# Vicky-Lamperouge/dlsa

Measured on AMD Instinct MI355X. Metric: DLSA logistic fit rows/sec (node), n=1e8 p=100, 1/2/4/8 GPUs; HBM GB/s, higher is better.
Workload: dtype f64

## Files before the change

### dlsa_amd/csrc/irls_oz_impl.hpp

```cpp
#pragma once

#include <stdint.h>
#include <stdlib.h>

#include <array>
#include <utility>

#include "dlsa_internal.hpp"
#include "wave_math.hpp"

namespace dlsa {

typedef int oz_i4 __attribute__((ext_vector_type(4)));

namespace ozk {

constexpr int NPW = 4;
constexpr int NCW = 4;
constexpr int RB = 32;
constexpr int RPW = RB / NPW;
constexpr int NSLOT = 6;
static_assert(NSLOT >= 6, "2 blocks in flight + 2 producing + 2 consuming");
#ifndef DLSA_OZ_CHECK
#define DLSA_OZ_CHECK 0
#endif
constexpr int ND = 5;
constexpr int GBITS = 38;
constexpr int NL = 5;
constexpr int EMIN = -985;
constexpr int EMAX = 1009;
constexpr double MAGIC = 6755399441055744.0 + 551911719040.0;

__host__ __device__ constexpr int xspan(int p) { return (RB * p * 8 + 16 + 15) & ~15; }
__host__ __device__ constexpr int npieces(int p) { return (xspan(p) + 1023) / 1024; }
__host__ __device__ constexpr int slot_bytes(int p) { return 16 + xspan(p) + 256; }
constexpr int kFeatBytes = 48;
constexpr int kMaxPiecesPerWave = 7;
__host__ __device__ constexpr int plane_off(int d) { return 8 * d; }
#ifndef DLSA_OZ_ABLATE
#define DLSA_OZ_ABLATE 0
#endif
__host__ __device__ constexpr int img_bytes(int NT) { return 16 * NT * kFeatBytes; }
__host__ __device__ constexpr int extra_bytes(int NT) { return 3 * 16 * NT * 8 + 16 * NT * 4; }
__host__ __device__ constexpr int lds_bytes(int NT, int p) {
  return NSLOT * slot_bytes(p) + extra_bytes(NT);
}
__host__ __device__ constexpr bool fits(int NT, int p) {
  return img_bytes(NT) <= RPW * p * 8 && lds_bytes(NT, p) <= 160 * 1024 &&
         npieces(p) <= NCW * kMaxPiecesPerWave;
}

constexpr unsigned strip_mask(int NT, int cw) {
  int load[NCW] = {0, 0, 0, 0};
  unsigned m[NCW] = {0, 0, 0, 0};
  for (int J = 0; J < NT; ++J) {
    int best = 0;
    for (int w = 1; w < NCW; ++w)
      if (load[w] < load[best]) best = w;
    load[best] += NT - J;
    m[best] |= 1u << J;
  }
  return m[cw];
}

template <int NT, int CW>
struct Tiles {
  static constexpr unsigned SM = strip_mask(NT, CW);
  static constexpr int count() {
    int c = 0;
    for (int J = 0; J < NT; ++J)
      if ((SM >> J) & 1u) c += NT - J;
    return c;
  }
  static constexpr int TW = count();
  static constexpr int index(int I, int J) {
    int c = 0;
    for (int j = 0; j < NT; ++j)
      if ((SM >> j) & 1u) {
        if (j == J) return c + (I - J);
        c += NT - j;
      }
    return -1;
  }
  static constexpr int I_of(int i) {
    for (int j = 0; j < NT; ++j)
      if ((SM >> j) & 1u) {
        if (i < NT - j) return j + i;
        i -= NT - j;
      }
    return -1;
  }
  static constexpr int J_of(int i) {
    for (int j = 0; j < NT; ++j)
      if ((SM >> j) & 1u) {
        if (i < NT - j) return j;
        i -= NT - j;
      }
    return -1;
  }
  static constexpr int strip_ordinal(int J) {
    int c = 0;
    for (int j = 0; j < J; ++j) c += (SM >> j) & 1u;
    return c;
  }
};

__device__ __forceinline__ uint32_t perm(uint32_t a, uint32_t b, uint32_t sel) {
  return __builtin_amdgcn_perm(a, b, sel);
}

__device__ __forceinline__ double level_value(const oz_i4 (&L)[NL], int r) {
  double v = (double)L[NL - 1][r];
#pragma unroll
  for (int k = NL - 2; k >= 0; --k) v = fma(v, 0x1p-8, (double)L[k][r]);
  return v;
}

__device__ __forceinline__ double xbound(uint32_t hi) {
  return __hiloint2double((int)(hi & 0x7FFFFFFFu), (int)0xFFFFFFFFu);
}
__device__ __forceinline__ int digit_exponent(uint32_t xhi, uint32_t zbits, double growth) {
  const double xb = xbound(xhi);
  const double zb = (double)__uint_as_float(zbits & 0x7FFFFFFFu) * (1.0 + 0x1p-16);
  double bound = fmax(fmax(zb, 0x1p-120), xb * 0x1p-60) * growth;
  bound = fmin(bound, 0.5 * xb);
  const int e = __builtin_amdgcn_frexp_exp(bound);
  return max(e, EMIN);
}
__device__ __forceinline__ bool digit_overflow(int e) { return e > EMAX; }

}

#ifdef DLSA_OZ_PROF
static __device__ unsigned long long g_oz_prof[32];
static inline int oz_prof_read_impl(unsigned long long* out) {
  if (hipDeviceSynchronize() != hipSuccess) return -1;
  if (hipMemcpyFromSymbol(out, HIP_SYMBOL(g_oz_prof), 32 * 8) != hipSuccess) return -1;
  unsigned long long z[32] = {0};
  return hipMemcpyToSymbol(HIP_SYMBOL(g_oz_prof), z, 32 * 8) == hipSuccess ? 0 : -1;
}
#define OZ_STAMP(v) const uint64_t v = __builtin_readcyclecounter()
#define OZ_STAMP_VAR(v) uint64_t v = 0
#define OZ_STAMP_SET(v) v = __builtin_readcyclecounter()
#define OZ_ADD(i, d) prof[i] += (d)
#define OZ_DECL uint64_t prof[4] = {0, 0, 0, 0}
#define OZ_FLUSH(base)                                                        \
  if (lane == 0)                                                              \
    for (int i_ = 0; i_ < 4; ++i_) atomicAdd(&g_oz_prof[(base) + i_], prof[i_])
#else
#define OZ_STAMP(v)
#define OZ_STAMP_VAR(v)
#define OZ_STAMP_SET(v)
#define OZ_ADD(i, d)
#define OZ_DECL
#define OZ_FLUSH(base)
#endif

template <int NT, int CW>
struct OzConsumer {
  using TL = ozk::Tiles<NT, CW>;
  static constexpr int TW = TL::TW;
  static constexpr int PMAX = 16 * NT;
  oz_i4 acc[TW > 0 ? TW : 1][ozk::NL];

  __device__ __forceinline__ void init() {
    static_for<(TW > 0 ? TW : 1)>([&](auto iI) {
      constexpr int i = decltype(iI)::value;
#pragma unroll
      for (int k = 0; k < ozk::NL; ++k) acc[i][k] = oz_i4{0, 0, 0, 0};
    });
  }

  template <typename Tick>
  __device__ __forceinline__ void consume(const char* xs, int p, int lane, Tick&& tick) {
    if constexpr (TW > 0) {
      const int i = lane & 15, g = lane >> 4;
      const char* im = xs + g * ozk::RPW * p * 8 + i * ozk::kFeatBytes;
      using u2 = unsigned __attribute__((ext_vector_type(2)));
      oz_i4 A0[2], A2[2];
      u2 A4[2];
      u2 Bd[2][ozk::ND];
      auto loadB = [&](auto jJ, int u) {
        constexpr int fo = 16 * decltype(jJ)::value * ozk::kFeatBytes;
#pragma unroll
        for (int b = 0; b < ozk::ND; ++b) Bd[u][b] = *(const u2*)(im + fo + 8 * b);
      };
      auto loadA = [&](auto tI, int u) {
        constexpr int fa = 16 * TL::I_of(decltype(tI)::value) * ozk::kFeatBytes;
        A0[u] = *(const oz_i4*)(im + fa);
        A2[u] = *(const oz_i4*)(im + fa + 16);
        A4[u] = *(const u2*)(im + fa + 32);
      };
      loadB(std::integral_constant<int, TL::J_of(0)>{}, 0);
      loadA(std::integral_constant<int, 0>{}, 0);
      static_for<TW>([&](auto tI) {
        constexpr int t = decltype(tI)::value;
        constexpr int J = TL::J_of(t);
        constexpr int ua = t & 1;
        constexpr int ub = TL::strip_ordinal(J) & 1;
        if constexpr (t + 1 < TW) {
          constexpr int Jn = TL::J_of(t + 1);
          if constexpr (Jn != J) loadB(std::integral_constant<int, Jn>{}, ub ^ 1);
          loadA(std::integral_constant<int, t + 1>{}, ua ^ 1);
        }
        __builtin_amdgcn_sched_barrier(0);
        const u2* d = Bd[ub];
        oz_i4 Bq[ozk::ND];
        Bq[0] = oz_i4{(int)d[0].x, (int)d[0].y, 0, 0};
#pragma unroll
        for (int b = 1; b < ozk::ND; ++b)
          Bq[b] = oz_i4{(int)d[b].x, (int)d[b].y, (int)d[b - 1].x, (int)d[b - 1].y};
        const oz_i4 a0 = A0[ua], a2 = A2[ua];
        const oz_i4 a4 = oz_i4{(int)A4[ua].x, (int)A4[ua].y, 0, 0};
        acc[t][0] = __builtin_amdgcn_mfma_i32_16x16x64_i8(a0, Bq[0], acc[t][0], 0, 0, 0);
        acc[t][1] = __builtin_amdgcn_mfma_i32_16x16x64_i8(a0, Bq[1], acc[t][1], 0, 0, 0);
        acc[t][2] = __builtin_amdgcn_mfma_i32_16x16x64_i8(a0, Bq[2], acc[t][2], 0, 0, 0);
        acc[t][3] = __builtin_amdgcn_mfma_i32_16x16x64_i8(a0, Bq[3], acc[t][3], 0, 0, 0);
        acc[t][4] = __builtin_amdgcn_mfma_i32_16x16x64_i8(a0, Bq[4], acc[t][4], 0, 0, 0);
        acc[t][2] = __builtin_amdgcn_mfma_i32_16x16x64_i8(a2, Bq[0], acc[t][2], 0, 0, 0);
        acc[t][3] = __builtin_amdgcn_mfma_i32_16x16x64_i8(a2, Bq[1], acc[t][3], 0, 0, 0);
        acc[t][4] = __builtin_amdgcn_mfma_i32_16x16x64_i8(a2, Bq[2], acc[t][4], 0, 0, 0);
        acc[t][4] = __builtin_amdgcn_mfma_i32_16x16x64_i8(a4, Bq[0], acc[t][4], 0, 0, 0);
        __builtin_amdgcn_sched_barrier(0);
        tick(std::integral_constant<int, t>{});
      });
      static_for<TW>([this](auto iI) {
        constexpr int t = decltype(iI)::value;
#pragma unroll
        for (int k = 0; k < ozk::NL; ++k) asm volatile("" : "+v"(acc[t][k]));
      });
    }
  }

  __device__ __forceinline__ void store(double* sH, const int* ex, int lane) {
    if constexpr (TW > 0) {
      const int fl = lane & 15, q = lane >> 4;
      static_for<TW>([&](auto iI) {
        constexpr int t = decltype(iI)::value;
        constexpr int I = TL::I_of(t), J = TL::J_of(t);
        constexpr int ts = I * (I + 1) / 2 + J;
        const int ej = ex[16 * J + fl];
#pragma unroll
        for (int r = 0; r < 4; ++r) {
          const int row = 4 * q + r;
          const double v = ozk::level_value(acc[t], r);
          sH[ts * 256 + row * 16 + fl] = __builtin_amdgcn_ldexp(v, ej + ex[16 * I + row] - 12);
        }
      });
    }
  }
};

template <int NT, bool STD, typename SlotX, typename Dma>
__device__ __forceinline__ void oz_producer(const PassArgs& a, char* smem, int wid, int lane,
                                            int tid, int nb, int nit, int sbytes, int xs_bytes,
                                            SlotX&& slot_x, const double* bet,
                                            const double* stdv, const int* ex, int chunk,
                                            bool chunk_ovf, Dma&& issue_pair) {
  using namespace ozk;
  constexpr int PMAX = 16 * NT;
  const int p = a.p, P = a.P, ic = a.intercept;
  const int nrows = __builtin_amdgcn_readfirstlane(a.chunk_rows[blockIdx.x]);
  const int pw = wid;
  const int q = lane >> 4, s = lane & 15;
  const int Xq = q >> 1, hq = q & 1;
  const int rbase = pw * RPW + 4 * hq;
  const bool up8 = s >= 8, up4 = ((s >> 2) & 1) != 0;
  const int myrow = s >> 2;
  double beta[NT], gacc[NT], mg[NT];
#pragma unroll
  for (int k = 0; k < NT; ++k) {
    const int f = 16 * k + s;
    beta[k] = bet[f];
    mg[k] = __builtin_amdgcn_ldexp(MAGIC, ex[f] - GBITS);
    gacc[k] = 0.0;
  }
  const bool fin_last = 16 * (NT - 1) + s < P;
  double llacc = 0.0, lprod = 1.0;

  issue_pair(-1);
  wait_vmcnt<0>();
  OZ_DECL;
  for (int m = 0; m < nit; ++m) {
    OZ_STAMP(t0);
    wait_vmcnt<0>();
    lds_barrier();
    OZ_STAMP(t1);
    OZ_ADD(0, t1 - t0);
    issue_pair(m);
    if (2 * m >= nb || (DLSA_OZ_ABLATE & 1)) continue;
    const int b = 2 * m + Xq;
    char* xq = slot_x(b);
    const double* yq = (const double*)(smem + (b % NSLOT) * sbytes + 16 + xs_bytes);
    const int leftq = nrows - b * RB;
    const bool full = nrows - 2 * m * RB >= 2 * RB;
    double v[4][NT], e[4];
    auto row_phase = [&](auto maskI) {
      constexpr bool MASK = decltype(maskI)::value;
#pragma unroll
      for (int r = 0; r < 4; ++r) {
        const int rowB = rbase + r;
        const bool valid = rowB < leftq;
        const double* xr = (const double*)xq + rowB * p + (s - ic);
        double er = 0.0;
#pragma unroll
        for (int k = 0; k < NT; ++k) {
          const int f = 16 * k + s;
          double x = xr[16 * k];
          if constexpr (DLSA_OZ_CHECK) {
            const int el = rowB * p + f - ic;
            if (f >= ic && f < P && (el < pw * RPW * p || el >= (pw + 1) * RPW * p))
              x = __builtin_nan("");
          }
          if constexpr (STD) x = (x - stdv[f]) * stdv[PMAX + f];
          if (k == 0 && ic && s == 0) x = 1.0;
          const bool fin = k < NT - 1 || fin_last;
          if constexpr (MASK)
            x = (valid && fin) ? x : 0.0;
          else
            x = fin ? x : 0.0;
          v[r][k] = x;
          er = fma(x, beta[k], er);
        }
        e[r] = er;
      }
    };
    if (full)
      row_phase(std::false_type{});
    else
      row_phase(std::true_type{});
    double e01, e23;
    {
      const double s0 = up8 ? e[0] : e[2], s1 = up8 ? e[1] : e[3];
      const double k0 = up8 ? e[2] : e[0], k1 = up8 ? e[3] : e[1];
      e01 = k0 + dpp_f64<0x128>(s0);
      e23 = k1 + dpp_f64<0x128>(s1);
    }
    double eh;
    {
      const double sn = up4 ? e01 : e23, kp = up4 ? e23 : e01;
      eh = kp + dpp_f64<0x141>(sn);
    }
    eh += dpp_f64<0xB1>(eh);
    eh += dpp_f64<0x4E>(eh);
    double swh, rh;
    {
      const bool valid = rbase + myrow < leftq;
      const double yv = valid ? yq[rbase + myrow] : 0.0;
      const double eqv = exp(-0.5 * fabs(eh));
      const double ea = eqv * eqv;
      const double inv = wv_rcp(1.0 + ea);
      const double mu = eh >= 0.0 ? inv : ea * inv;
      swh = eqv * inv;
      rh = yv - mu;
      if (valid && (s & 3) == 0) {
        llacc += yv * eh - fmax(eh, 0.0);
        lprod *= 1.0 + ea;
      }
      if (!valid) {
        swh = 0.0;
        rh = 0.0;
      }
    }
    double sw[4], res[4];
    sw[0] = dpp_f64<0x150>(swh);
    sw[1] = dpp_f64<0x154>(swh);
    sw[2] = dpp_f64<0x158>(swh);
    sw[3] = dpp_f64<0x15C>(swh);
    res[0] = dpp_f64<0x150>(rh);
    res[1] = dpp_f64<0x154>(rh);
    res[2] = dpp_f64<0x158>(rh);
    res[3] = dpp_f64<0x15C>(rh);
    OZ_STAMP(t2);
    OZ_ADD(1, t2 - t1);
    char* img = xq + pw * RPW * p * 8 + 4 * hq;
#pragma unroll
    for (int k = 0; k < NT; ++k) {
      gacc[k] = fma(v[0][k], res[0], gacc[k]);
      gacc[k] = fma(v[1][k], res[1], gacc[k]);
      gacc[k] = fma(v[2][k], res[2], gacc[k]);
      gacc[k] = fma(v[3][k], res[3], gacc[k]);
      uint32_t lo[4], hi[4];
#pragma unroll
      for (int r = 0; r < 4; ++r) {
        const double t = fma(v[r][k], sw[r], mg[k]);
        lo[r] = __double2loint(t);
        hi[r] = __double2hiint(t);
      }
      const uint32_t u01 = perm(lo[1], lo[0], 0x05010400u), w01 = perm(lo[1], lo[0], 0x07030602u);
      const uint32_t u23 = perm(lo[3], lo[2], 0x05010400u), w23 = perm(lo[3], lo[2], 0x07030602u);
      const uint32_t d4 = perm(u23, u01, 0x05040100u) ^ 0x80808080u;
      const uint32_t d3 = perm(u23, u01, 0x07060302u) ^ 0x80808080u;
      const uint32_t d2 = perm(w23, w01, 0x05040100u) ^ 0x80808080u;
      const uint32_t d1 = perm(w23, w01, 0x07060302u) ^ 0x80808080u;
      const uint32_t d0 = perm(perm(hi[3], hi[2], 0x05010400u), perm(hi[1], hi[0], 0x05010400u),
                               0x05040100u) ^ 0x80808080u;
      char* fe = img + (16 * k + s) * kFeatBytes;
      *(uint32_t*)(fe + plane_off(0)) = d0;
      *(uint32_t*)(fe + plane_off(1)) = d1;
      *(uint32_t*)(fe + plane_off(2)) = d2;
      *(uint32_t*)(fe + plane_off(3)) = d3;
      *(uint32_t*)(fe + plane_off(4)) = d4;
    }
#ifdef DLSA_OZ_PROF
    asm volatile("s_waitcnt lgkmcnt(0)" ::: "memory");
#endif
    OZ_STAMP(t3);
    OZ_ADD(2, t3 - t2);
  }
  OZ_FLUSH(4 * pw);
  __syncthreads();

  double* red = (double*)smem;
#pragma unroll
  for (int k = 0; k < NT; ++k) {
    double g = gacc[k];
    g += __shfl_xor(g, 16);
    g += __shfl_xor(g, 32);
    if (q == 0) red[pw * (PMAX + 1) + 16 * k + s] = g;
  }
  llacc -= log(lprod);
#pragma unroll
  for (int o = 1; o < 64; o <<= 1) llacc += __shfl_xor(llacc, o);
  if (lane == 0) red[pw * (PMAX + 1) + PMAX] = llacc;
  __syncthreads();
  for (int f = tid; f < PMAX; f += 64 * NPW) {
    double sg = 0.0;
#pragma unroll
    for (int w = 0; w < NPW; ++w) sg += red[w * (PMAX + 1) + f];
    a.slab_g[(int64_t)chunk * PMAX + f] = sg;
  }
  if (tid == 0) {
    double sg = 0.0;
#pragma unroll
    for (int w = 0; w < NPW; ++w) sg += red[w * (PMAX + 1) + PMAX];
    a.slab_ll[chunk] = chunk_ovf ? __builtin_nan("") : sg;
  }
}

template <int NT, bool STD>
__global__ __launch_bounds__(64 * (ozk::NPW + ozk::NCW), 1) void irls_oz_kernel(const PassArgs a) {
  using namespace ozk;
  constexpr int PMAX = 16 * NT;
  extern __shared__ __attribute__((aligned(16))) char smem[];

  const int chunk = blockIdx.x;
  const int part = __builtin_amdgcn_readfirstlane(a.chunk_part[chunk]);
  if (a.phase[part] != a.want_phase) return;

  const int tid = threadIdx.x;
  const int lane = tid & 63;
  const int wid = __builtin_amdgcn_readfirstlane(tid >> 6);
  const int p = a.p, P = a.P, ic = a.intercept;
  const int64_t row0 = uniform_row0(a.chunk_row0, chunk);
  const int nrows = __builtin_amdgcn_readfirstlane(a.chunk_rows[chunk]);
  const int nb = (nrows + RB - 1) / RB;
  const int nit = (nb + 1) / 2 + 1;
  const int sbytes = slot_bytes(p);
  const int np = npieces(p);
  const int xs_bytes = xspan(p);
  double* bet = (double*)(smem + NSLOT * sbytes);
  double* stdv = bet + PMAX;
  int* ex = (int*)(stdv + 2 * PMAX);

  double dth = 0.0;
  uint32_t xh = 0;
  bool e_ovf = false;
  if (tid < PMAX) {
    const double th = (tid < P) ? a.theta[(int64_t)part * P + tid] : 0.0;
    bet[tid] = th;
    if (tid < P) dth = fabs(th - a.theta_rec[(int64_t)part * P + tid]);
    xh = a.colmax[(int64_t)chunk * PMAX + tid] & 0x7FFFFFFFu;
    if constexpr (STD) {
      const int j = tid - ic;
      const bool in = j >= 0 && j < p;
      stdv[tid] = in ? a.center[j] : 0.0;
      stdv[PMAX + tid] = in ? 1.0 / a.scale[j] : 1.0;
    }
  }
#pragma unroll
  for (int o = 1; o < 64; o <<= 1) {
    dth += __shfl_xor(dth, o);
    xh = max(xh, (uint32_t)__shfl_xor((int)xh, o));
  }
  double* dred = (double*)smem;
  uint32_t* xred = (uint32_t*)(dred + (NPW + NCW));
  if (lane == 0) {
    dred[wid] = dth;
    xred[wid] = xh;
  }
  __syncthreads();
  if (tid < PMAX) {
    double sd = 0.0;
    uint32_t xm = 0;
#pragma unroll
    for (int w = 0; w < NPW + NCW; ++w) {
      sd += dred[w];
      xm = max(xm, xred[w]);
    }
    const double growth = exp(0.5 * sd * ozk::xbound(xm)) * (1.0 + 0x1p-40);
    const int e = digit_exponent(a.colmax[(int64_t)chunk * PMAX + tid],
                                 a.zcolmax[(int64_t)chunk * PMAX + tid], growth);
    ex[tid] = min(e, ozk::EMAX);
    if (wid == 0) {
      e_ovf = ozk::digit_overflow(e);
      if (tid + 64 < PMAX)
        e_ovf = e_ovf || ozk::digit_overflow(digit_exponent(
                             a.colmax[(int64_t)chunk * PMAX + tid + 64],
                             a.zcolmax[(int64_t)chunk * PMAX + tid + 64], growth));
    }
  }
  const bool chunk_ovf = wid == 0 && __ballot(e_ovf) != 0;
  __syncthreads();

  auto slot_x = [&](int blk) -> char* {
    const uintptr_t start = (uintptr_t)(a.X + (row0 + (int64_t)blk * RB) * p);
    return smem + (blk % NSLOT) * sbytes + 16 + (start & 15);
  };

  constexpr int KP = 1;
  const int dw = wid >= NPW ? wid - NPW : wid;
  const uintptr_t xcb = (uintptr_t)(a.X + row0 * p) & ~(uintptr_t)15;
  const __amdgpu_buffer_rsrc_t xr = uniform_rsrc(xcb, a.x_last16 + 16 - xcb);
  const uintptr_t ycb = (uintptr_t)(a.y + row0);
  const __amdgpu_buffer_rsrc_t yr = uniform_rsrc(ycb, a.y_last4 + 4 - ycb);
  const int npw = (np - dw + NCW - 1) / NCW;
  auto blk_lds = [&](int blk) { return __builtin_amdgcn_readfirstlane((blk % NSLOT) * sbytes); };
  auto blk_soff = [&](int blk) {
    const uintptr_t start = (uintptr_t)(a.X + (row0 + (int64_t)blk * RB) * p);
    return __builtin_amdgcn_readfirstlane((int)((start & ~(uintptr_t)15) - xcb));
  };
  auto issue_x = [&](auto iI, int lds, int soff) {
    constexpr int i = decltype(iI)::value;
    if (i < npw) {
      const int j = dw + NCW * i;
      const int off = j == np - 1 ? xs_bytes - 1024 : j * 1024;
      __builtin_amdgcn_raw_ptr_buffer_load_lds(xr, (lds_void_t*)(smem + lds + 16 + off), 16,
                                               lane * 16, soff + off, 0, DLSA_OZ_DMA_AUX);
    }
  };
  auto issue_y = [&](int blk, int lds) {
    if (dw == NCW - 1)
      __builtin_amdgcn_raw_ptr_buffer_load_lds(yr, (lds_void_t*)(smem + lds + 16 + xs_bytes), 4,
                                               lane * 4, blk * RB * 8, 0, 0);
  };
  auto issue_rest = [&](auto I0, int blk, int lds, int soff) {
    static_for<kMaxPiecesPerWave>([&](auto iI) {
      if constexpr (decltype(iI)::value >= decltype(I0)::value) issue_x(iI, lds, soff);
    });
    issue_y(blk, lds);
  };
  static_assert(KP == 1, "issue_pair issues piece 0 only");
  auto issue_pair = [&](int m) {
#pragma unroll
    for (int X = 2; X < 4; ++X) {
      const int blk = 2 * m + X;
      if (blk < nb) issue_x(std::integral_constant<int, 0>{}, blk_lds(blk), blk_soff(blk));
    }
  };

  if (wid >= NPW) {
    const int cw = wid - NPW;
    auto run = [&](auto cwI) {
      constexpr int CW = decltype(cwI)::value;
      constexpr int TW = OzConsumer<NT, CW>::TW;
      __builtin_amdgcn_s_setprio(1);
      OzConsumer<NT, CW> C;
      C.init();
      for (int b = 0; b < 2 && b < nb; ++b)
        issue_rest(std::integral_constant<int, KP>{}, b, blk_lds(b), blk_soff(b));
      wait_vmcnt<0>();
      OZ_DECL;
      for (int m = 0; m < nit; ++m) {
        OZ_STAMP(t0);
        lds_barrier();
        OZ_STAMP(t1);
        const bool d0 = 2 * m + 2 < nb, d1 = 2 * m + 3 < nb;
        const int l0 = blk_lds(2 * m + 2), s0 = blk_soff(2 * m + 2);
        const int l1 = blk_lds(2 * m + 3), s1 = blk_soff(2 * m + 3);
        const bool c0 = m >= 1 && !(DLSA_OZ_ABLATE & 2);
        const bool c1 = c0 && 2 * m - 1 < nb;
        OZ_STAMP_VAR(t2);
        auto tickA = [&](auto tI) {
          constexpr int i = KP + decltype(tI)::value;
          if (d0) issue_x(std::integral_constant<int, i>{}, l0, s0);
          if (d1) issue_x(std::integral_constant<int, i>{}, l1, s1);
        };
        auto tickN = [&](auto) {};
        if (c0) C.consume(slot_x(2 * m - 2), p, lane, tickA);
        if (c0) {
          if (d0) issue_rest(std::integral_constant<int, KP + TW>{}, 2 * m + 2, l0, s0);
          if (d1) issue_rest(std::integral_constant<int, KP + TW>{}, 2 * m + 3, l1, s1);
        } else {
          if (d0) issue_rest(std::integral_constant<int, KP>{}, 2 * m + 2, l0, s0);
          if (d1) issue_rest(std::integral_constant<int, KP>{}, 2 * m + 3, l1, s1);
        }
        if (c1) C.consume(slot_x(2 * m - 1), p, lane, tickN);
        OZ_STAMP_SET(t2);
        OZ_STAMP(t3);
        wait_vmcnt<0>();
        OZ_STAMP(t4);
        OZ_ADD(0, t1 - t0);
        OZ_ADD(1, t3 - t2);
        OZ_ADD(2, t2 - t1);
        OZ_ADD(3, t4 - t3);
      }
      OZ_FLUSH(4 * (NPW + CW));
      __syncthreads();
      C.store(a.slab_H + (int64_t)chunk * (NT * (NT + 1) / 2) * 256, ex, lane);
      __syncthreads();
    };
    switch (cw) {
      case 0: run(std::integral_constant<int, 0>{}); break;
      case 1: run(std::integral_constant<int, 1>{}); break;
      case 2: run(std::integral_constant<int, 2>{}); break;
      default: run(std::integral_constant<int, 3>{}); break;
    }
    return;
  }

  oz_producer<NT, STD>(a, smem, wid, lane, tid, nb, nit, sbytes, xs_bytes, slot_x, bet, stdv,
                       ex, chunk, chunk_ovf, issue_pair);
}

template <int NT, bool STD>
static hipError_t launch_oz_t(const PassArgs& a, int n_chunks, hipStream_t s) {
  auto kern = irls_oz_kernel<NT, STD>;
  hipError_t e = ensure_max_lds((const void*)kern, 160 * 1024);
  if (e != hipSuccess) return e;
  hipLaunchKernelGGL(kern, dim3(n_chunks), dim3(64 * (ozk::NPW + ozk::NCW)),
                     ozk::lds_bytes(NT, a.p), s, a);
  return hipGetLastError();
}

template <int NT>
static hipError_t launch_oz_nt(const PassArgs& a, bool std_, int n_chunks, hipStream_t s) {
  return std_ ? launch_oz_t<NT, true>(a, n_chunks, s) : launch_oz_t<NT, false>(a, n_chunks, s);
}

typedef hipError_t OzUnitFn(const PassArgs& a, int NT, bool std_, int family, int n_chunks,
                            hipStream_t s);
#define DLSA_OZ_UNIT(name, ...)                                                                  \
  hipError_t name(const PassArgs& a, int NT, bool std_, int family, int n_chunks, hipStream_t s) { \
    return unit_dispatch(FamLogistic{}, IntList<__VA_ARGS__>{}, family, NT, [&](auto, auto nt) { \
      return launch_oz_nt<decltype(nt)::value>(a, std_, n_chunks, s);                            \
    });                                                                                          \
  }

}
```

Before: 1.328 billion.

## Consume two row blocks per MFMA pass by pairing slots into 128-bit operands

The consumer now reads each digit plane from two adjacent LDS slots with explicit ds_read_b64 pairs and packs them into one 128-bit MFMA operand, so a single consume call covers both blocks of the pair instead of two separate consume calls. The MFMA product list is rewritten for full 5x5 digit pairs up to total order 4, and lgkmcnt waits are made explicit. The prefetch schedule issues four pieces up front (KP=4) instead of one. This aims to halve consume overhead and improve MFMA K utilisation, at the cost of more registers and hand-written asm waits that bypass compiler scheduling.

```diff
diff --git a/dlsa_amd/csrc/irls_oz_impl.hpp b/dlsa_amd/csrc/irls_oz_impl.hpp
--- a/dlsa_amd/csrc/irls_oz_impl.hpp
+++ b/dlsa_amd/csrc/irls_oz_impl.hpp
@@ -172,24 +172,41 @@
   }
 
   template <typename Tick>
-  __device__ __forceinline__ void consume(const char* xs, int p, int lane, Tick&& tick) {
+  __device__ __forceinline__ void consume(const char* xs, int sb, int p, int lane, Tick&& tick) {
     if constexpr (TW > 0) {
       const int i = lane & 15, g = lane >> 4;
       const char* im = xs + g * ozk::RPW * p * 8 + i * ozk::kFeatBytes;
+      const char* im1 = im + sb;
       using u2 = unsigned __attribute__((ext_vector_type(2)));
-      oz_i4 A0[2], A2[2];
-      u2 A4[2];
-      u2 Bd[2][ozk::ND];
+      const uint32_t a0 = (uint32_t)(uintptr_t)(const lds_void_t*)im, a1 = a0 + sb;
+      oz_i4 Ad[2][ozk::ND], Bd[2][ozk::ND];
+      auto plane = [&](auto offI) {
+        constexpr int off = decltype(offI)::value;
+        static_assert(off >= 0 && off < 65536, "ds_read_b64 takes a 16-bit byte offset");
+        u2 e, o;
+        asm volatile("ds_read_b64 %0, %1 offset:%2" : "=v"(e) : "v"(a0), "n"(off) : "memory");
+        asm volatile("ds_read_b64 %0, %1 offset:%2" : "=v"(o) : "v"(a1), "n"(off) : "memory");
+        return oz_i4{(int)e.x, (int)e.y, (int)o.x, (int)o.y};
+      };
+      auto load_planes = [&](oz_i4* q, auto foI) {
+        static_for<ozk::ND>([&](auto dI) {
+          constexpr int d = decltype(dI)::value;
+          q[d] = plane(std::integral_constant<int, decltype(foI)::value + ozk::plane_off(d)>{});
+        });
+      };
+      auto wait_planes = [&](oz_i4* a, oz_i4* b) {
+        static_assert(ozk::ND == 5, "the operand list below");
+        asm volatile("s_waitcnt lgkmcnt(0)"
+                     : "+v"(a[0]), "+v"(a[1]), "+v"(a[2]), "+v"(a[3]), "+v"(a[4]), "+v"(b[0]),
+                       "+v"(b[1]), "+v"(b[2]), "+v"(b[3]), "+v"(b[4]));
+      };
       auto loadB = [&](auto jJ, int u) {
-        constexpr int fo = 16 * decltype(jJ)::value * ozk::kFeatBytes;
-#pragma unroll
-        for (int b = 0; b < ozk::ND; ++b) Bd[u][b] = *(const u2*)(im + fo + 8 * b);
+        load_planes(Bd[u],
+                    std::integral_constant<int, 16 * decltype(jJ)::value * ozk::kFeatBytes>{});
       };
       auto loadA = [&](auto tI, int u) {
-        constexpr int fa = 16 * TL::I_of(decltype(tI)::value) * ozk::kFeatBytes;
-        A0[u] = *(const oz_i4*)(im + fa);
-        A2[u] = *(const oz_i4*)(im + fa + 16);
-        A4[u] = *(const u2*)(im + fa + 32);
+        load_planes(Ad[u], std::integral_constant<int, 16 * TL::I_of(decltype(tI)::value) *
+                                                           ozk::kFeatBytes>{});
       };
       loadB(std::integral_constant<int, TL::J_of(0)>{}, 0);
       loadA(std::integral_constant<int, 0>{}, 0);
@@ -198,29 +215,34 @@
         constexpr int J = TL::J_of(t);
         constexpr int ua = t & 1;
         constexpr int ub = TL::strip_ordinal(J) & 1;
+        wait_planes(Ad[ua], Bd[ub]);
         if constexpr (t + 1 < TW) {
           constexpr int Jn = TL::J_of(t + 1);
           if constexpr (Jn != J) loadB(std::integral_constant<int, Jn>{}, ub ^ 1);
           loadA(std::integral_constant<int, t + 1>{}, ua ^ 1);
         }
         __builtin_amdgcn_sched_barrier(0);
-        const u2* d = Bd[ub];
-        oz_i4 Bq[ozk::ND];
-        Bq[0] = oz_i4{(int)d[0].x, (int)d[0].y, 0, 0};
-#pragma unroll
-        for (int b = 1; b < ozk::ND; ++b)
-          Bq[b] = oz_i4{(int)d[b].x, (int)d[b].y, (int)d[b - 1].x, (int)d[b - 1].y};
-        const oz_i4 a0 = A0[ua], a2 = A2[ua];
-        const oz_i4 a4 = oz_i4{(int)A4[ua].x, (int)A4[ua].y, 0, 0};
-        acc[t][0] = __builtin_amdgcn_mfma_i32_16x16x64_i8(a0, Bq[0], acc[t][0], 0, 0, 0);
-        acc[t][1] = __builtin_amdgcn_mfma_i32_16x16x64_i8(a0, Bq[1], acc[t][1], 0, 0, 0);
-        acc[t][2] = __builtin_amdgcn_mfma_i32_16x16x64_i8(a0, Bq[2], acc[t][2], 0, 0, 0);
-        acc[t][3] = __builtin_amdgcn_mfma_i32_16x16x64_i8(a0, Bq[3], acc[t][3], 0, 0, 0);
-        acc[t][4] = __builtin_amdgcn_mfma_i32_16x16x64_i8(a0, Bq[4], acc[t][4], 0, 0, 0);
-        acc[t][2] = __builtin_amdgcn_mfma_i32_16x16x64_i8(a2, Bq[0], acc[t][2], 0, 0, 0);
-        acc[t][3] = __builtin_amdgcn_mfma_i32_16x16x64_i8(a2, Bq[1], acc[t][3], 0, 0, 0);
-        acc[t][4] = __builtin_amdgcn_mfma_i32_16x16x64_i8(a2, Bq[2], acc[t][4], 0, 0, 0);
-        acc[t][4] = __builtin_amdgcn_mfma_i32_16x16x64_i8(a4, Bq[0], acc[t][4], 0, 0, 0);
+        const oz_i4* A = Ad[ua];
+        const oz_i4* B = Bd[ub];
+#define DLSA_OZ_MFMA(a_, b_) \
+  acc[t][a_ + b_] = __builtin_amdgcn_mfma_i32_16x16x64_i8(A[a_], B[b_], acc[t][a_ + b_], 0, 0, 0)
+        DLSA_OZ_MFMA(0, 0);
+        DLSA_OZ_MFMA(0, 1);
+        DLSA_OZ_MFMA(0, 2);
+        DLSA_OZ_MFMA(0, 3);
+        DLSA_OZ_MFMA(0, 4);
+        DLSA_OZ_MFMA(1, 0);
+        DLSA_OZ_MFMA(1, 1);
+        DLSA_OZ_MFMA(1, 2);
+        DLSA_OZ_MFMA(1, 3);
+        DLSA_OZ_MFMA(2, 0);
+        DLSA_OZ_MFMA(4, 0);
+        DLSA_OZ_MFMA(2, 1);
+        DLSA_OZ_MFMA(2, 2);
+        DLSA_OZ_MFMA(3, 0);
+        DLSA_OZ_MFMA(3, 1);
+#undef DLSA_OZ_MFMA
+        static_assert(ozk::NL == 5 && ozk::ND == 5, "the product list above");
         __builtin_amdgcn_sched_barrier(0);
         tick(std::integral_constant<int, t>{});
       });
@@ -518,7 +540,7 @@
     return smem + (blk % NSLOT) * sbytes + 16 + (start & 15);
   };
 
-  constexpr int KP = 1;
+  constexpr int KP = 4;
   const int dw = wid >= NPW ? wid - NPW : wid;
   const uintptr_t xcb = (uintptr_t)(a.X + row0 * p) & ~(uintptr_t)15;
   const __amdgpu_buffer_rsrc_t xr = uniform_rsrc(xcb, a.x_last16 + 16 - xcb);
@@ -532,7 +554,7 @@
   };
   auto issue_x = [&](auto iI, int lds, int soff) {
     constexpr int i = decltype(iI)::value;
-    if (i < npw) {
+    if (i < kMaxPiecesPerWave && i < npw) {
       const int j = dw + NCW * i;
       const int off = j == np - 1 ? xs_bytes - 1024 : j * 1024;
       __builtin_amdgcn_raw_ptr_buffer_load_lds(xr, (lds_void_t*)(smem + lds + 16 + off), 16,
@@ -550,12 +572,12 @@
     });
     issue_y(blk, lds);
   };
-  static_assert(KP == 1, "issue_pair issues piece 0 only");
   auto issue_pair = [&](int m) {
 #pragma unroll
     for (int X = 2; X < 4; ++X) {
       const int blk = 2 * m + X;
-      if (blk < nb) issue_x(std::integral_constant<int, 0>{}, blk_lds(blk), blk_soff(blk));
+      if (blk < nb)
+        static_for<KP>([&](auto iI) { issue_x(iI, blk_lds(blk), blk_soff(blk)); });
     }
   };
 
@@ -579,23 +601,20 @@
         const int l0 = blk_lds(2 * m + 2), s0 = blk_soff(2 * m + 2);
         const int l1 = blk_lds(2 * m + 3), s1 = blk_soff(2 * m + 3);
         const bool c0 = m >= 1 && !(DLSA_OZ_ABLATE & 2);
-        const bool c1 = c0 && 2 * m - 1 < nb;
         OZ_STAMP_VAR(t2);
-        auto tickA = [&](auto tI) {
+        auto tick = [&](auto tI) {
           constexpr int i = KP + decltype(tI)::value;
           if (d0) issue_x(std::integral_constant<int, i>{}, l0, s0);
           if (d1) issue_x(std::integral_constant<int, i>{}, l1, s1);
         };
-        auto tickN = [&](auto) {};
-        if (c0) C.consume(slot_x(2 * m - 2), p, lane, tickA);
         if (c0) {
+          C.consume(slot_x(2 * m - 2), sbytes, p, lane, tick);
           if (d0) issue_rest(std::integral_constant<int, KP + TW>{}, 2 * m + 2, l0, s0);
           if (d1) issue_rest(std::integral_constant<int, KP + TW>{}, 2 * m + 3, l1, s1);
         } else {
           if (d0) issue_rest(std::integral_constant<int, KP>{}, 2 * m + 2, l0, s0);
           if (d1) issue_rest(std::integral_constant<int, KP>{}, 2 * m + 3, l1, s1);
         }
-        if (c1) C.consume(slot_x(2 * m - 1), p, lane, tickN);
         OZ_STAMP_SET(t2);
         OZ_STAMP(t3);
         wait_vmcnt<0>();
```

Result: no change. 1.339 billion (median of 6 runs) (+0.8%).
